# stardist/stardist

Measured on AMD Instinct MI355X. Metric: predict_instances() Mpix/s (2D) + Mvox/s (3D) end-to-end at 1/2/4/8 GPU, higher is better.
Workload: dtype f32

## Files before the change

include/stardist_hip.h:

```cpp
#ifndef STARDIST_HIP_H
#define STARDIST_HIP_H

#include <stdbool.h>
#include <stdint.h>

#ifdef __cplusplus
extern "C" {
#endif

const char* sd_last_error(void);
int sd_version(void);
int sd_device_count(void);
int sd_release_workspace(void);
int sd_set_option(const char* name, int value);
int sd_get_option(const char* name);

int sd_nms2d_host(const float* dist, const float* points, int n_polys, int n_rays,
                  int use_kdtree, int use_bbox, int verbose, float threshold,
                  uint8_t* keep, int64_t* stats);
int sd_nms2d_device(const float* d_dist, const float* d_points, int n_polys, int n_rays,
                    int use_kdtree, int use_bbox, int verbose, float threshold,
                    uint8_t* d_keep, int64_t* stats, void* stream);

int sd_nms2d_build_device(const float* d_dist, const float* d_points, int n_polys, int n_rays, int32_t* d_vx, int32_t* d_vy,
                          int32_t* d_bbox, float* d_radius, float* d_area, int32_t* d_gstats, void* stream);

int sd_nms2d_old_host(const int32_t* polys, int n_polys, int n_rays, const int32_t* mapping, int height, int width,
                      float threshold, int max_bbox_search, int grid_y, int grid_x, int verbose, uint8_t* keep);
int sd_nms2d_old_device(const int32_t* d_polys, int n_polys, int n_rays, const int32_t* d_mapping, int height, int width,
                        float threshold, int max_bbox_search, int grid_y, int grid_x, int verbose, uint8_t* d_keep, void* stream);

int sd_prepare_polys_device(const int32_t* d_x, const int32_t* d_y, int n_polys, int n_verts, void* d_out,
                            int64_t out_bytes, void* stream);

int sd_clip_pairs_device(const int32_t* d_xa, const int32_t* d_ya, const int32_t* d_xb,
                         const int32_t* d_yb, int n_pairs, int n_verts,
                         int64_t* d_out_twice_area, int32_t* d_out_flags, void* stream);

int sd_area_bounds_pairs_device(const int32_t* d_xa, const int32_t* d_ya, const int32_t* d_xb, const int32_t* d_yb, int n_pairs,
                                int n_verts, float* d_out_area, float* d_out_band, int32_t* d_out_info, void* stream);

int sd_poly_pass_device(const int32_t* d_x, const int32_t* d_y, int n_polys, int n_verts, void* d_props, void* d_prep, void* stream);

int sd_star_dist2d_host(const uint16_t* src, int H, int W, int n_rays, int grid_y, int grid_x,
                        float* dst);
int sd_star_dist2d_device(const uint16_t* d_src, int H, int W, int n_rays, int grid_y,
                          int grid_x, float* d_dst, void* stream);
int sd_star_dist3d_host(const uint16_t* src, int Z, int Y, int X, const float* dz,
                        const float* dy, const float* dx, int n_rays, int grid_z, int grid_y,
                        int grid_x, float* dst);
int sd_star_dist3d_device(const uint16_t* d_src, int Z, int Y, int X, const float* d_dz,
                          const float* d_dy, const float* d_dx, int n_rays, int grid_z,
                          int grid_y, int grid_x, float* d_dst, void* stream);

int sd_edt_prob_device(const int32_t* d_lbl, int Z, int Y, int X, double sz, double sy, double sx, int max_label,
                       float* d_prob, void* stream);

int sd_polygons_to_label_host(const float* coord, const int32_t* labels, int n_polys, int n_rays,
                              int H, int W, int32_t* result);
int sd_polygons_to_label_device(const float* d_coord, const int32_t* d_labels, int n_polys,
                                int n_rays, int H, int W, int32_t* d_result, void* stream);
int sd_polygons_to_label_window_device(const float* d_coord, const int32_t* d_labels, int n_polys, int n_rays, int HI, int WI,
                                       int y0, int x0, int H, int W, int32_t* d_result, void* stream);
// ... 182 lines not shown
```

stardist_amd/csrc/area_bounds.h:

```cpp
#pragma once
#include <hip/hip_runtime.h>

namespace sdarea {

enum { PP_PLAIN = 1, PP_POS = 2, PP_NEG = 4 };
struct PolyProps { float lmax, perim; int flags; int xmin, xmax, ymin, ymax; int pad; };

__device__ __forceinline__ float sgnf(float v) { return v > 0.f ? 1.f : (v < 0.f ? -1.f : 0.f); }
__device__ __forceinline__ float half_sum(float v) { for (int o = 16; o; o >>= 1) v += __shfl_xor(v, o); return v; }
__device__ __forceinline__ float half_max(float v) { for (int o = 16; o; o >>= 1) v = fmaxf(v, __shfl_xor(v, o)); return v; }
__device__ __forceinline__ int half_sum_i(int v) { for (int o = 16; o; o >>= 1) v += __shfl_xor(v, o); return v; }
__device__ __forceinline__ int half_min_i(int v) { for (int o = 16; o; o >>= 1) { const int t = __shfl_xor(v, o); v = t < v ? t : v; } return v; }
__device__ __forceinline__ int half_max_i(int v) { for (int o = 16; o; o >>= 1) { const int t = __shfl_xor(v, o); v = t > v ? t : v; } return v; }

constexpr float NEAR_W = 0.15f, STRIP_W = 0.45f;
constexpr int WINDOW = 2047;


struct Enclosure { float area, band; int crossings, near; bool usable; };

__device__ __forceinline__ Enclosure pair_enclosure(const int* __restrict__ px, const int* __restrict__ py, const int* __restrict__ qx,
                                                    const int* __restrict__ qy, int R, const PolyProps& pp, const PolyProps& pq, bool active,
                                                    float2* sq, int l, int half) {
  Enclosure E; E.area = 0.f; E.band = 0.f; E.crossings = 0; E.near = 0; E.usable = false;
  const int hb = half << 5;
  bool use = active && (pp.flags & PP_PLAIN) && (pq.flags & PP_PLAIN) && ((pp.flags & (PP_POS | PP_NEG)) == (pq.flags & (PP_POS | PP_NEG)));
  const int ox = use ? (int)(((long long)pp.xmin + pp.xmax) >> 1) : 0, oy = use ? (int)(((long long)pp.ymin + pp.ymax) >> 1) : 0;
  long long ext = 0;
  if (use) {
    const long long e0 = (long long)pp.xmax - ox, e1 = (long long)ox - pp.xmin, e2 = (long long)pp.ymax - oy, e3 = (long long)oy - pp.ymin;
    const long long e4 = (long long)pq.xmax - ox, e5 = (long long)ox - pq.xmin, e6 = (long long)pq.ymax - oy, e7 = (long long)oy - pq.ymin;
    ext = e0; ext = e1 > ext ? e1 : ext; ext = e2 > ext ? e2 : ext; ext = e3 > ext ? e3 : ext;
    ext = e4 > ext ? e4 : ext; ext = e5 > ext ? e5 : ext; ext = e6 > ext ? e6 : ext; ext = e7 > ext ? e7 : ext;
    if (ext > WINDOW / 2) use = false;
  }
  const bool lv = use && l < R;
  float ax = 0.f, ay = 0.f, cqx = 0.f, cqy = 0.f;
  if (lv) { ax = (float)(px[l] - ox); ay = (float)(py[l] - oy); cqx = (float)(qx[l] - ox); cqy = (float)(qy[l] - oy); }
  sq[l] = make_float2(cqx, cqy);
  const int ln = (l + 1 >= R) ? 0 : l + 1;
  const float bx = __shfl(ax, hb + ln), by = __shfl(ay, hb + ln);
  __builtin_amdgcn_wave_barrier();
  const float ex = bx - ax, ey = by - ay;
  const bool oke = lv && (ex != 0.f || ey != 0.f);
  const bool tie_e_pos = ey != 0.f ? ey < 0.f : ex > 0.f;
  const bool e_up = by > ay;
  const bool sPpos = (pp.flags & PP_POS) != 0, sQpos = (pq.flags & PP_POS) != 0;
  const float exlo = fminf(ax, bx) - 1.f, exhi = fmaxf(ax, bx) + 1.f, eylo = fminf(ay, by) - 1.f, eyhi = fmaxf(ay, by) + 1.f;
  float accP = 0.f, accQ = 0.f;
  int K = 0, T = 0, parA = 0, SQ = 0;
  bool nearP = false;
  float2 c = sq[0];
  float o_ec = ex * (c.y - ay) - ey * (c.x - ax);
  const int Rw = __any(use) ? R : 0;
  for (int k = 0; k < Rw; ++k) {
    const int kn = (k + 1 >= R) ? 0 : k + 1;
    const float2 d = sq[kn];
    const float fx = d.x - c.x, fy = d.y - c.y;
    const bool okf = use & ((fx != 0.f) | (fy != 0.f));
    const bool tie_f_pos = fy != 0.f ? fy > 0.f : fx < 0.f;
    const float o_ed = ex * (d.y - ay) - ey * (d.x - ax);
    const float o_fa = fx * (ay - c.y) - fy * (ax - c.x), o_fb = fx * (by - c.y) - fy * (bx - c.x);
    const bool pos_c = (o_ec > 0.f) | ((o_ec == 0.f) & tie_e_pos), pos_d = (o_ed > 0.f) | ((o_ed == 0.f) & tie_e_pos);
    const bool pos_a = (o_fa > 0.f) | ((o_fa == 0.f) & tie_f_pos), pos_b = (o_fb > 0.f) | ((o_fb == 0.f) & tie_f_pos);
    const float ccd = c.x * d.y - c.y * d.x;
    const bool both = oke & okf;
    const bool nearb = both & ((c.x <= exhi) | (d.x <= exhi)) & ((c.x >= exlo) | (d.x >= exlo)) & ((c.y <= eyhi) | (d.y <= eyhi)) & ((c.y >= eylo) | (d.y >= eylo));
    T += nearb ? 1 : 0;
    nearP |= nearb;
    {
      const unsigned long long nb64 = __ballot(nearb);
      SQ += ((unsigned int)(half ? (nb64 >> 32) : nb64) != 0u) ? 1 : 0;
    }
    if (both & (pos_c != pos_d) & (pos_a != pos_b)) {
      const float t = o_fa * __builtin_amdgcn_rcpf(o_fa - o_fb), u = o_ec * __builtin_amdgcn_rcpf(o_ec - o_ed);
      const float wt = 1.f - t, wu = 1.f - u;
      accP += (pos_b == sQpos) ? wt : -wt;
      accQ += ccd * ((pos_d == sPpos) ? wu : -wu);
      ++K;
    }
    parA ^= (okf & ((c.y < ay) != (d.y < ay)) & (pos_a == (fy > 0.f))) ? 1 : 0;
    const bool hitC = oke & use & ((ay <= c.y) != (by <= c.y)) & (pos_c == e_up);
    const unsigned long long hb64 = __ballot(hitC);
    const unsigned int hm = (unsigned int)(half ? (hb64 >> 32) : hb64);
    if ((__popc(hm) & 1) && l == 0) accQ += ccd;
    c = d; o_ec = o_ed;
  }
  const float cab = ax * by - ay * bx;
  const float contrib = lv ? cab * ((float)parA + accP) + accQ : 0.f;
  const float tot = half_sum(contrib);
  const int Kt = half_sum_i(lv ? K : 0), Tt = half_sum_i(lv ? T : 0), SPt = half_sum_i((lv && nearP) ? 1 : 0);
  const int St = SPt > SQ ? SPt : SQ;
  E.area = 0.5f * fabsf(tot);
  E.crossings = Kt; E.near = Tt;
  E.band = (0.5f * (float)Kt + fmaxf(NEAR_W * (float)Tt, STRIP_W * (float)St)) * (pp.lmax + pq.lmax) + 0.75f + 2e-6f * (float)ext * (pp.perim + pq.perim);
  if (use) {
    long long M = 0;
    const long long a0 = pp.xmin < 0 ? -(long long)pp.xmin : pp.xmin, a1 = pp.xmax < 0 ? -(long long)pp.xmax : pp.xmax;
    const long long a2 = pp.ymin < 0 ? -(long long)pp.ymin : pp.ymin, a3 = pp.ymax < 0 ? -(long long)pp.ymax : pp.ymax;
    const long long b0 = pq.xmin < 0 ? -(long long)pq.xmin : pq.xmin, b1 = pq.xmax < 0 ? -(long long)pq.xmax : pq.xmax;
    const long long b2 = pq.ymin < 0 ? -(long long)pq.ymin : pq.ymin, b3 = pq.ymax < 0 ? -(long long)pq.ymax : pq.ymax;
    M = (a0 > a1 ? a0 : a1); M = b0 > M ? b0 : M; M = b1 > M ? b1 : M;
    long long My = (a2 > a3 ? a2 : a3); My = b2 > My ? b2 : My; My = b3 > My ? b3 : My;
    const double bound = (double)(M + My + 2) * ((double)pp.perim + (double)pq.perim + 3.0 * Kt + 4.0);
    if (!(bound < 16777216.0)) use = false;
  }
  E.usable = use;
  return E;
}

__device__ __forceinline__ int decide(const Enclosure& E, float area_i, float area_j, float thr) {
  if (!E.usable) return 0;
  const double amin = fmin((double)area_i + 1.e-10, (double)area_j + 1.e-10);
  if (!(amin > 0.25)) return 0;
  const double lo = ((double)E.area - (double)E.band) / amin, hi = ((double)E.area + (double)E.band) / amin;
  const double m = 4e-6 * fabs((double)thr) + 1e-6;
  if (lo > (double)thr + m) return 2;
  if (hi < (double)thr - m) return 1;
  return 0;
}

}
```

stardist_amd/csrc/area_bounds.hip:

```cpp
#include "common.h"
#include "area_bounds.h"
#include "poly_pass.h"
#include "../../include/stardist_hip.h"

namespace {
__global__ void __launch_bounds__(256) k_area_probe(const int* __restrict__ xa, const int* __restrict__ ya, const int* __restrict__ xb,
                                                    const int* __restrict__ yb, int n, int R, const sdarea::PolyProps* __restrict__ pa,
                                                    const sdarea::PolyProps* __restrict__ pb, float* __restrict__ out_area, float* __restrict__ out_band,
                                                    int* __restrict__ out_info) {
  __shared__ float2 sq[4][2][32];
  const int lane = threadIdx.x & 63, half = lane >> 5, l = lane & 31, wv = threadIdx.x >> 6;
  const long long nw = (long long)gridDim.x * 4;
  for (long long base = 2ll * ((long long)blockIdx.x * 4 + wv); base < n; base += 2ll * nw) {
    const long long t = base + half;
    const bool active = t < n;
    const long long tt = active ? t : 0;
    const sdarea::Enclosure E = sdarea::pair_enclosure(xa + tt * R, ya + tt * R, xb + tt * R, yb + tt * R, R, pa[tt], pb[tt], active, sq[wv][half], l, half);
    if (active && l == 0) { out_area[t] = E.area; out_band[t] = E.band; out_info[t] = (E.usable ? 1 : 0) | ((E.crossings & 0x3FF) << 8) | ((E.near & 0x7FF) << 18); }
    __builtin_amdgcn_wave_barrier();
  }
}
}

extern "C" int sd_area_bounds_pairs_device(const int32_t* d_xa, const int32_t* d_ya, const int32_t* d_xb, const int32_t* d_yb, int n_pairs, int n_verts,
                                           float* d_out_area, float* d_out_band, int32_t* d_out_info, void* stream) {
  hipStream_t s = (hipStream_t)stream;
  if (n_pairs <= 0) return 0;
  const int R = n_verts;
  if (R < 3 || R > 32) { sd::set_error("sd_area_bounds_pairs: n_verts=%d unsupported (3..32)", R); return -1; }
  sd::Arena& A = sd::arena();
  if (A.begin(s)) return -1;
  sdarea::PolyProps* pa = (sdarea::PolyProps*)A.take((size_t)n_pairs * sizeof(sdarea::PolyProps));
  sdarea::PolyProps* pb = (sdarea::PolyProps*)A.take((size_t)n_pairs * sizeof(sdarea::PolyProps));
  if (!pa || !pb) return -1;
  if (sdpass::launch_poly_pass(d_xa, d_ya, n_pairs, R, pa, nullptr, s) || sdpass::launch_poly_pass(d_xb, d_yb, n_pairs, R, pb, nullptr, s)) {
    sd::set_error("sd_area_bounds_pairs: launch failed");
    return -1;
  }
  const int blocks = sd::div_up(n_pairs, 8) < 2048 ? sd::div_up(n_pairs, 8) : 2048;
  hipLaunchKernelGGL(k_area_probe, dim3(blocks), dim3(256), 0, s, d_xa, d_ya, d_xb, d_yb, n_pairs, R, pa, pb, d_out_area, d_out_band, d_out_info);
  SD_LAUNCH_CHECK();
  SD_CHECK(hipStreamSynchronize(s));
  return 0;
}

extern "C" int sd_poly_pass_device(const int32_t* d_x, const int32_t* d_y, int n_polys, int n_verts, void* d_props, void* d_prep, void* stream) {
  hipStream_t s = (hipStream_t)stream;
  if (n_polys <= 0 || (!d_props && !d_prep)) return 0;
  const int R = n_verts;
  if (R < (d_props ? 3 : 1) || R > 32) { sd::set_error("sd_poly_pass: n_verts=%d unsupported (%d..32)", R, d_props ? 3 : 1); return -1; }
  if (sdpass::launch_poly_pass(d_x, d_y, n_polys, R, (sdarea::PolyProps*)d_props, d_prep, s)) { sd::set_error("sd_poly_pass: launch failed"); return -1; }
  SD_CHECK(hipStreamSynchronize(s));
  return 0;
}
```

stardist_amd/csrc/common.h:

```cpp
#pragma once
#include <hip/hip_runtime.h>
#include <stdint.h>
#include <stdio.h>
#include <string.h>

namespace sd {

char* err_buf();
void set_error(const char* fmt, ...);

#define SD_CHECK(expr)                                                                   \
  do {                                                                                   \
    hipError_t _e = (expr);                                                              \
    if (_e != hipSuccess) {                                                              \
      sd::set_error("%s:%d: %s -> %s", __FILE__, __LINE__, #expr, hipGetErrorString(_e)); \
      return -1;                                                                         \
    }                                                                                    \
  } while (0)

#define SD_LAUNCH_CHECK() SD_CHECK(hipGetLastError())

class Arena {
 public:
  int begin(hipStream_t stream);
  void* take(size_t bytes);
  template <typename T> T* take_n(size_t n) { return (T*)take((n ? n : 1) * sizeof(T)); }
  void release();
  size_t capacity() const;
 private:
  enum { kMaxChunks = 64 };
  void* base_[kMaxChunks] = {};
  size_t cap_[kMaxChunks] = {};
  int n_ = 0, cur_ = 0;
  size_t off_ = 0;
};
Arena& arena();

hipStream_t side_stream();

static inline int div_up(long long a, long long b) { return (int)((a + b - 1) / b); }

enum Option { OPT_NMS3D_VOLUME_BOUNDS, OPT_NMS3D_CONE_MAP, OPT_NMS3D_REFINE_MESH, OPT_PROBE_TIER, OPT_PROBE_NO_GENERAL, OPT_TRACE, OPT_NMS3D_TAIL_BATCH, OPT_NMS3D_SPLIT_EXACT, OPT_CONV_F16_WGS, OPT_NMS2D_PAIR_LANES, OPT_NMS2D_AREA_BOUNDS, OPT_NMS2D_DEFER_UNDECIDED, OPT_NMS2D_STRICT, OPT_NMS2D_NBR_SINGLE, OPT_NMS3D_NBR_SINGLE, OPT_NMS2D_DEFER_MAX, OPT_NMS3D_BOUNDS_REUSE, OPT_NMS3D_DEFER_EXACT, OPT_NMS3D_BOUNDS_LEAN, OPT_COUNT };
int option(Option o);

#ifdef SD_DEBUG_SWITCHES
int tuning_env(const char* name, int dflt);
#else
static inline int tuning_env(const char*, int dflt) { return dflt; }
#endif

}
```

stardist_amd/csrc/lib.hip:

```cpp
#include "common.h"
#include "../../include/stardist_hip.h"
#include <stdarg.h>
#include <stdlib.h>
#include <mutex>

namespace sd {

static thread_local char g_err[1024] = "";
char* err_buf() { return g_err; }
void set_error(const char* fmt, ...) {
  va_list ap;
  va_start(ap, fmt);
  vsnprintf(g_err, sizeof(g_err), fmt, ap);
  va_end(ap);
}

static int g_opt[OPT_COUNT] = {1, 1, 2, 1, 0, 0, 1, 3, 2, 64, 1, 2, 0, 1, 1, 16384, 1, 3, 1};
static const char* const g_opt_name[OPT_COUNT] = {"nms3d_volume_bounds", "nms3d_cone_map", "nms3d_refine_mesh", "probe_tier", "probe_no_general", "trace", "nms3d_tail_batch", "nms3d_split_exact", "conv_f16_workgroups_per_cu", "nms2d_pair_lanes", "nms2d_area_bounds", "nms2d_defer_undecided", "nms2d_strict", "nms2d_neighbours_single_pass", "nms3d_neighbours_single_pass", "nms2d_defer_max", "nms3d_bounds_reuse", "nms3d_defer_exact", "nms3d_bounds_lean"};
int option(Option o) { return g_opt[o]; }
#ifdef SD_DEBUG_SWITCHES
int tuning_env(const char* name, int dflt) { const char* e = getenv(name); return e ? atoi(e) : dflt; }
#endif

enum { kMaxDevices = 64 };
static Arena g_arena[kMaxDevices];
Arena& arena() {
  int d = 0;
  if (hipGetDevice(&d) != hipSuccess || d < 0 || d >= kMaxDevices) d = 0;
  return g_arena[d];
}

hipStream_t side_stream() {
  static std::mutex mu;
  static hipStream_t st[kMaxDevices] = {};
  int d = 0;
  if (hipGetDevice(&d) != hipSuccess || d < 0 || d >= kMaxDevices) { set_error("side_stream: no current device"); return nullptr; }
  std::lock_guard<std::mutex> lock(mu);
  if (!st[d] && hipStreamCreateWithFlags(&st[d], hipStreamNonBlocking) != hipSuccess) { st[d] = nullptr; set_error("side_stream: cannot create a stream"); }
  return st[d];
}

size_t Arena::capacity() const { size_t t = 0; for (int i = 0; i < n_; ++i) t += cap_[i]; return t; }
int Arena::begin(hipStream_t stream) {
  if (n_ > 1) {
    size_t total = capacity();
    SD_CHECK(hipStreamSynchronize(stream));
    for (int i = 0; i < n_; ++i) { (void)hipFree(base_[i]); base_[i] = nullptr; cap_[i] = 0; }
    n_ = 0;
    size_t want = total + (total >> 3);
    SD_CHECK(hipMalloc(&base_[0], want));
    cap_[0] = want; n_ = 1;
  }
  cur_ = 0; off_ = 0;
  return 0;
}
void* Arena::take(size_t bytes) {
  for (;;) {
    if (cur_ < n_) {
      size_t a = (off_ + 255) & ~size_t(255);
      if (a + bytes <= cap_[cur_]) { off_ = a + bytes; return (char*)base_[cur_] + a; }
      ++cur_; off_ = 0;
      continue;
// ... 38 lines not shown
```

stardist_amd/csrc/nms2d.hip:

```cpp
#include <type_traits>

#include "common.h"
#include "clip_sweep.h"
#include "clip_beam.h"
#include "area_bounds.h"
#include "poly_pass.h"
#include "nms_rounds.h"
#include "../../include/stardist_hip.h"
#include <hipcub/hipcub.hpp>
#include <math.h>
#include <stdlib.h>
#include <vector>

namespace {

using sdclip::i64;

__device__ __forceinline__ float wave_min(float v) { for (int o = 32; o; o >>= 1) v = fminf(v, __shfl_xor(v, o)); return v; }
__device__ __forceinline__ float wave_max(float v) { for (int o = 32; o; o >>= 1) v = fmaxf(v, __shfl_xor(v, o)); return v; }
__device__ __forceinline__ i64 wave_sum(i64 v) { for (int o = 32; o; o >>= 1) v += __shfl_xor(v, o); return v; }

__global__ void __launch_bounds__(256) k_build(const float* __restrict__ dist, const float* __restrict__ pts,
                                               const float2* __restrict__ sincos, int N, int R,
                                               int* __restrict__ vx, int* __restrict__ vy, int4* __restrict__ bbox,
// ... 375 lines not shown
      continue;
    }
    if ((st & ~sdclip::ST_FAIL) || bm.n_joins > 0 || bm.sum_abs_terms >= (1ll << 24)) {
      const unsigned int k = atomicAdd(q.exactCount, 1u);
      if (k < q.cap) q.exact[k] = p;
      continue;
    }
    const float area_inter = 0.5f * (float)twice;
    const float overlap = (float)((double)area_inter / fmin((double)area[ij.x] + 1.e-10, (double)area[ij.y] + 1.e-10));
    if (overlap > thr) { if (supp) supp[p] = 1; else state[ij.y] = ST_SUPPRESSED; }
  }
}
template <int MAXV, int K, int MAXIL, int MAXREC, int S, bool REL16 = false>
size_t beam_lds_bytes() {
  typedef typename std::conditional<REL16, sdclip::LdsStorage16<S>, sdclip::LdsStorage<S>>::type Storage;
  return (size_t)sdclip::Beam<MAXV, K, MAXIL, MAXREC, Storage>::lds_bytes() + 64;
}

__global__ void __launch_bounds__(256) k_pairs_decide(const int2* __restrict__ pairs, const unsigned long long* __restrict__ nPtr,
                                                      const unsigned int* __restrict__ firstPtr, const int* __restrict__ vx, const int* __restrict__ vy, int R,
                                                      const sdarea::PolyProps* __restrict__ props, const float* __restrict__ area, float thr,
                                                      unsigned char* __restrict__ state, unsigned char* __restrict__ supp,
                                                      unsigned char* __restrict__ decided, unsigned int* __restrict__ nDecided) {
  __shared__ float2 sq[4][2][32];
  const int lane = threadIdx.x & 63, half = lane >> 5, l = lane & 31, wv = threadIdx.x >> 6;
  const unsigned long long n = *nPtr, first = firstPtr ? (unsigned long long)*firstPtr : 0ull;
  const unsigned long long nw = (unsigned long long)gridDim.x * 4;
  unsigned int mine = 0;
  for (unsigned long long base = first + 2ull * ((unsigned long long)blockIdx.x * 4 + wv); base < n; base += 2ull * nw) {
    const unsigned long long t = base + half;
    const bool active = t < n;
    const int2 ij = active ? pairs[t] : make_int2(0, 0);
    const sdarea::PolyProps pp = props[ij.x], pq = props[ij.y];
    const sdarea::Enclosure E = sdarea::pair_enclosure(vx + (size_t)ij.x * R, vy + (size_t)ij.x * R, vx + (size_t)ij.y * R, vy + (size_t)ij.y * R, R, pp, pq,
                                                       active, sq[wv][half], l, half);
    if (active && l == 0) {
      const int dec = sdarea::decide(E, area[ij.x], area[ij.y], thr);
      decided[t] = (unsigned char)dec;
      if (dec == 2) { if (supp) supp[t] = 1; else state[ij.y] = ST_SUPPRESSED; }
      if (dec) ++mine;
    }
    __builtin_amdgcn_wave_barrier();
  }
  mine += __shfl_xor(mine, 32);
  if (lane == 0 && mine) atomicAdd(nDecided, mine);
}

__global__ void __launch_bounds__(256) k_tail_emit(const int* __restrict__ U, int nU, const unsigned char* __restrict__ state,
                                                   const i64* __restrict__ nbrStart, const int* __restrict__ nbrLow, const int* __restrict__ nbr, NmsFlags f,
                                                   const float* __restrict__ pts, const int4* __restrict__ bbox,
                                                   const float* __restrict__ radius, const float* __restrict__ area,
                                                   int2* __restrict__ pairs, unsigned long long* pairCount, unsigned long long pairCap,
                                                   unsigned int* __restrict__ segStart, int* __restrict__ segCnt) {
  const int wave = threadIdx.x >> 6, lane = threadIdx.x & 63;
  for (int w = blockIdx.x * (blockDim.x >> 6) + wave; w < nU; w += gridDim.x * (blockDim.x >> 6)) {
    const int j = U[w];
    int cnt = 0;
    unsigned long long base = 0;
// ... 470 lines not shown
  const int* nbr = L.nbr;
  int* waitOn = L.waitOn;
  const i64 totalNbr = 2 * L.total;

  SD_CHECK(hipStreamWaitEvent(s, evProps, 0));
  if (stats) { SD_CHECK(hipEventRecord(ev1, s)); SD_CHECK(hipEventSynchronize(ev1)); float ms = 0; SD_CHECK(hipEventElapsedTime(&ms, ev0, ev1)); ns_pre = ms * 1e6; }

  const unsigned long long pairCap = (unsigned long long)(totalNbr / 2 + 64);
  int* U1 = A.take_n<int>(N);
  int* K = A.take_n<int>(N);
  int2* pairs = A.take_n<int2>(pairCap);
  const unsigned int qCap = (unsigned int)(pairCap < (1ull << 30) ? pairCap : (1ull << 30));
  unsigned int* spillPairs = A.take_n<unsigned int>(qCap);
  unsigned int* exactPairs = A.take_n<unsigned int>(qCap);
  int* Sl = A.take_n<int>(N);
  Counters* d_cnt = (Counters*)A.take(sizeof(Counters));
  static const bool pairSort = sd::tuning_env("SD_NMS_PAIR_SORT", 1) != 0;
  unsigned int* pairOrder = pairSort && R <= 32 ? A.take_n<unsigned int>(qCap) : nullptr;
  unsigned int* bucketHist = A.take_n<unsigned int>(2 * PAIR_BUCKETS);
  unsigned long long* nOrdered = A.take_n<unsigned long long>(1);
  if (!U0 || !U1 || !K || !pairs || !spillPairs || !exactPairs || !Sl || !d_cnt || !bucketHist || !nOrdered || (pairSort && R <= 32 && !pairOrder)) return -1;
  unsigned char* decided = (areaBounds && pairOrder) ? A.take_n<unsigned char>(pairCap) : nullptr;
  if (areaBounds && pairOrder && !decided) return -1;
  i64 totalDecided = 0, totalSkipped = 0;
  int nU = N, rounds = 0;
  i64 totalPairs = 0, totalExact = 0, totalSpill = 0;
  int* Ucur = U0; int* Unext = U1;
  Counters h;
  hipEvent_t ev2 = nullptr, ev3 = nullptr;
  if (stats) { SD_CHECK(hipEventCreate(&ev2)); SD_CHECK(hipEventCreate(&ev3)); }
  EvGuard evguard2{ev2, ev3};
  static const int tailDiv = sd::tuning_env("SD_NMS_TAIL_DIV", 6);
  static const int tailMax = sd::tuning_env("SD_NMS_TAIL_MAX", 65536);
  const int tailT = tailDiv > 0 ? ((N / tailDiv) < tailMax ? (N / tailDiv) : tailMax) : -1;
  unsigned char* supp = nullptr; unsigned int* segStart = nullptr; int* segCnt = nullptr;
  static const bool deferEnv = sd::tuning_env("SD_NMS_DEFER", 1) != 0;
  const bool deferOn = tailT >= 0 && deferEnv;
  Deferred dfr{nullptr, nullptr, nullptr, nullptr, nullptr, qCap};
  unsigned int* firstNew = A.take_n<unsigned int>(1);
  dfr.pend = pend0; dfr.head = head0; dfr.count = dcount0;
  if (!firstNew) return -1;
  if (deferOn) {
    dfr.pairs = A.take_n<int2>(qCap);
    dfr.next = A.take_n<int>(qCap);
    if (!dfr.pairs || !dfr.next) return -1;
  }
// ... 5 lines not shown
  const unsigned int deferMax = (unsigned int)(sd::option(sd::OPT_NMS2D_DEFER_MAX) > 0 ? sd::option(sd::OPT_NMS2D_DEFER_MAX) : 0);
  unsigned char* defKind = nullptr; unsigned int* nJoinDef = nullptr;
  if (deferFrom > 0) {
    defKind = A.take_n<unsigned char>(qCap); nJoinDef = A.take_n<unsigned int>(1);
    if (!defKind || !nJoinDef) return -1;
    SD_CHECK(hipMemsetAsync(defKind, 0, qCap, s));
  }
  i64 totalUndecDeferred = 0;
  i64 nUndecDeferredUpper = 0;
  auto run_pairs = [&](unsigned char* suppOut) -> int {
    const unsigned int* first = suppOut ? firstNew : nullptr;
    if (stats) SD_CHECK(hipEventRecord(ev0, s));
    PairQueues q1{spillPairs, &d_cnt->nSpill, exactPairs, &d_cnt->nExact, qCap};
    PairQueues q2{exactPairs, &d_cnt->nExact, exactPairs, &d_cnt->nExact, qCap};
    int rc;
    if (R <= 32) {
      if (pairOrder) {
        static const int keyMode = sd::tuning_env("SD_NMS_PAIR_KEY", 2);
        static const int modes[6][3] = {{1, 32, 32}, {1, 64, 16}, {1, 64, 64}, {16, 16, 16}, {16, 32, 8}, {4, 32, 32}};
        const int* md = modes[keyMode >= 0 && keyMode < 6 ? keyMode : 2];
        const PairKey key{(const char*)prep, prepStride, 1.f / (4.f * (max_dist + 1.f)), md[0], md[1], md[2]};
        SD_CHECK(hipMemsetAsync(bucketHist, 0, PAIR_BUCKETS * sizeof(unsigned int), s));
        if (decided)
          hipLaunchKernelGGL(k_pairs_decide, dim3(256 * 8), dim3(256), 0, s, pairs, &d_cnt->nPairs, first, vx, vy, R, props, area, threshold, state, suppOut,
                             decided, &d_cnt->nDecided);
        if (!suppOut && deferFrom > 0 && rounds >= deferFrom)
          hipLaunchKernelGGL(k_defer_undecided, dim3(256), dim3(256), 0, s, pairs, &d_cnt->nPairs, &d_cnt->nDecided, deferMax, decided, state, dfr, defKind, &d_cnt->nErr);
        const unsigned int* bfirst = (suppOut && deferFrom > 0) ? nullptr : first;
        SD_CHECK(hipStreamWaitEvent(s, evPrep, 0));
        const unsigned char* liveState = suppOut ? nullptr : state;
        hipLaunchKernelGGL(k_pair_bucket_count, dim3(512), dim3(256), 0, s, pairs, &d_cnt->nPairs, bfirst, d_points, key, bucketHist, decided, liveState,
                           &d_cnt->nSkipped);
        hipLaunchKernelGGL(k_pair_bucket_scan, dim3(1), dim3(1024), 0, s, bucketHist, bucketHist + PAIR_BUCKETS, nOrdered);
        hipLaunchKernelGGL(k_pair_bucket_scatter, dim3(512), dim3(256), 0, s, pairs, &d_cnt->nPairs, bfirst, d_points, key, bucketHist + PAIR_BUCKETS,
                           pairOrder, qCap, decided, liveState);
        SD_LAUNCH_CHECK();
        rc = BeamPath<32, 64>::tier1(pairs, pairOrder, nOrdered, (const unsigned int*)nullptr, prep, area, threshold, state, suppOut, q1, s);
      } else {
        SD_CHECK(hipStreamWaitEvent(s, evPrep, 0));
        rc = BeamPath<32, 64>::tier1(pairs, (const unsigned int*)nullptr, &d_cnt->nPairs, first, prep, area, threshold, state, suppOut, q1, s);
      }
      if (stats) SD_CHECK(hipEventRecord(ev1, s));
      if (!rc) rc = BeamPath<32, 64>::tier2(pairs, spillPairs, &d_cnt->nSpill, (const unsigned int*)nullptr, prep, area, threshold, state, suppOut, q2, s);
    } else {
      SD_CHECK(hipStreamWaitEvent(s, evPrep, 0));
      if (R <= 64) rc = BeamPath<64, 64>::tier2(pairs, (const unsigned int*)nullptr, &d_cnt->nPairs, first, prep, area, threshold, state, suppOut, q2, s);
      else if (R <= 128) rc = BeamPath<128, 32>::tier2(pairs, (const unsigned int*)nullptr, &d_cnt->nPairs, first, prep, area, threshold, state, suppOut, q2, s);
// ... 323 lines not shown
```

stardist_amd/lib/_native.py:

```python
import ctypes
import os

import numpy as np

_HERE = os.path.dirname(os.path.abspath(__file__))
LIB_PATH = os.path.join(_HERE, "..", "csrc", "libstardist_hip.so")

_lib = None
last_stats = {}

_c_f32p = ctypes.POINTER(ctypes.c_float)
_c_i32p = ctypes.POINTER(ctypes.c_int32)
_c_i64p = ctypes.POINTER(ctypes.c_int64)
_c_u8p = ctypes.POINTER(ctypes.c_uint8)
_c_u16p = ctypes.POINTER(ctypes.c_uint16)
_vp = ctypes.c_void_p
_i = ctypes.c_int
_f = ctypes.c_float

SIGNATURES = {
    "sd_last_error": (ctypes.c_char_p, []),
    "sd_version": (_i, []),
    "sd_device_count": (_i, []),
    "sd_release_workspace": (_i, []),
    "sd_set_option": (_i, [ctypes.c_char_p, _i]),
    "sd_get_option": (_i, [ctypes.c_char_p]),
    "sd_nms2d_host": (_i, [_vp, _vp, _i, _i, _i, _i, _i, _f, _vp, _vp]),
    "sd_nms2d_device": (_i, [_vp, _vp, _i, _i, _i, _i, _i, _f, _vp, _vp, _vp]),
    "sd_nms2d_build_device": (_i, [_vp, _vp, _i, _i, _vp, _vp, _vp, _vp, _vp, _vp, _vp]),
    "sd_nms2d_old_host": (_i, [_vp, _i, _i, _vp, _i, _i, _f, _i, _i, _i, _i, _vp]),
    "sd_nms2d_old_device": (_i, [_vp, _i, _i, _vp, _i, _i, _f, _i, _i, _i, _i, _vp, _vp]),
    "sd_clip_pairs_device": (_i, [_vp, _vp, _vp, _vp, _i, _i, _vp, _vp, _vp]),
    "sd_area_bounds_pairs_device": (_i, [_vp, _vp, _vp, _vp, _i, _i, _vp, _vp, _vp, _vp]),
    "sd_prepare_polys_device": (_i, [_vp, _vp, _i, _i, _vp, ctypes.c_int64, _vp]),
    "sd_poly_pass_device": (_i, [_vp, _vp, _i, _i, _vp, _vp, _vp]),
    "sd_star_dist2d_host": (_i, [_vp, _i, _i, _i, _i, _i, _vp]),
    "sd_star_dist2d_device": (_i, [_vp, _i, _i, _i, _i, _i, _vp, _vp]),
    "sd_star_dist3d_host": (_i, [_vp, _i, _i, _i, _vp, _vp, _vp, _i, _i, _i, _i, _vp]),
    "sd_star_dist3d_device": (_i, [_vp, _i, _i, _i, _vp, _vp, _vp, _i, _i, _i, _i, _vp, _vp]),
    "sd_edt_prob_device": (_i, [_vp, _i, _i, _i, ctypes.c_double, ctypes.c_double, ctypes.c_double, _i, _vp, _vp]),
    "sd_dist_to_coord_device": (_i, [_vp, _vp, _vp, ctypes.c_longlong, _i, ctypes.c_double, ctypes.c_double, _vp, _vp]),
    "sd_polygons_to_label_host": (_i, [_vp, _vp, _i, _i, _i, _i, _vp]),
    "sd_polygons_to_label_device": (_i, [_vp, _vp, _i, _i, _i, _i, _vp, _vp]),
    "sd_polygons_to_label_window_device": (_i, [_vp, _vp, _i, _i, _i, _i, _i, _i, _i, _i, _vp, _vp]),
    "sd_polyhedron_to_label_window_device": (_i, [_vp, _vp, _vp, _vp, _i, _i, _i, _vp] + [_i] * 13 + [_vp, _vp]),
    "_LIB_non_maximum_suppression_sparse": (None, [_vp, _vp, _vp, _i, _i, _i, _vp, _vp, _f, _i, _i, _i, _vp]),
    "sd_nms3d_device": (_i, [_vp, _vp, _vp, _i, _i, _i, _vp, _vp, _f, _i, _i, _i, _vp, _vp, _vp]),
    "sd_hiv_pairs_device": (_i, [_vp, _vp, _i, _i, _i, _vp, _vp, _vp, _i, _vp, _vp, _vp]),
    "_LIB_polyhedron_to_label": (None, [_vp, _vp, _vp, _vp, _i, _i, _i, _vp, _i, _i, _i, _i, _i, _i, _i, _vp]),
    "sd_polyhedron_to_label_device": (_i, [_vp, _vp, _vp, _vp, _i, _i, _i, _vp, _i, _i, _i, _i, _i, _i, _i, _vp, _vp]),
    "sd_select_candidates_device": (_i, [_vp, _vp, _i, _vp, _vp, _i, _f, _i, _vp, _vp, _vp, _vp, _vp]),
    "sd_survivor_positions_device": (_i, [_vp, ctypes.c_longlong, _vp, _vp, _vp]),
    "sd_survivors2d_device": (_i, [_vp, _i, _vp, _vp, _vp, _i, _vp, _vp, _vp, _vp, _vp, _vp, _vp]),
    "sd_sorted_rows_device": (_i, [_vp, _vp, _i, _i, _vp, _vp, _vp, _vp, _vp, _vp, _vp]),
    "sd_sort_scores_desc_device": (_i, [_vp, _i, _vp, _vp, _vp]),
    "sd_bias_act_device": (_i, [_vp, _vp, ctypes.c_longlong, _i, ctypes.c_longlong, _i, _vp]),
# ... 138 lines not shown
```

Before: 322.0.

## Restructure pair enclosure inner loop with precomputed edge records and lane masks

```diff
diff --git a/include/stardist_hip.h b/include/stardist_hip.h
--- a/include/stardist_hip.h
+++ b/include/stardist_hip.h
@@ -39,6 +39,7 @@
 
 int sd_area_bounds_pairs_device(const int32_t* d_xa, const int32_t* d_ya, const int32_t* d_xb, const int32_t* d_yb, int n_pairs,
                                 int n_verts, float* d_out_area, float* d_out_band, int32_t* d_out_info, void* stream);
+int sd_area_bounds_pairs_grid(void);
 
 int sd_poly_pass_device(const int32_t* d_x, const int32_t* d_y, int n_polys, int n_verts, void* d_props, void* d_prep, void* stream);
 
diff --git a/stardist_amd/csrc/area_bounds.h b/stardist_amd/csrc/area_bounds.h
--- a/stardist_amd/csrc/area_bounds.h
+++ b/stardist_amd/csrc/area_bounds.h
@@ -19,90 +19,140 @@
 
 struct Enclosure { float area, band; int crossings, near; bool usable; };
 
-__device__ __forceinline__ Enclosure pair_enclosure(const int* __restrict__ px, const int* __restrict__ py, const int* __restrict__ qx,
-                                                    const int* __restrict__ qy, int R, const PolyProps& pp, const PolyProps& pq, bool active,
-                                                    float2* sq, int l, int half) {
+struct PairOperands { int word, px, py, qx, qy; };
+__device__ __forceinline__ PairOperands load_operands(const int* __restrict__ px, const int* __restrict__ py, const int* __restrict__ qx,
+                                                      const int* __restrict__ qy, const PolyProps* __restrict__ pp, const PolyProps* __restrict__ pq,
+                                                      bool live, int l) {
+  static_assert(sizeof(PolyProps) == 32, "eight words per record");
+  PairOperands o;
+  o.word = 0;
+  if (l < 16) o.word = (l < 8 ? (const int*)pp : (const int*)pq)[l & 7];
+  o.px = o.py = o.qx = o.qy = 0;
+  if (live) { o.px = px[l]; o.py = py[l]; o.qx = qx[l]; o.qy = qy[l]; }
+  return o;
+}
+__device__ __forceinline__ PolyProps props_from_lanes(int word, int first) {
+  PolyProps p;
+  p.lmax = __int_as_float(__shfl(word, first)); p.perim = __int_as_float(__shfl(word, first + 1)); p.flags = __shfl(word, first + 2);
+  p.xmin = __shfl(word, first + 3); p.xmax = __shfl(word, first + 4); p.ymin = __shfl(word, first + 5); p.ymax = __shfl(word, first + 6);
+  p.pad = 0;
+  return p;
+}
+
+typedef unsigned long long lanemask;
+__device__ __forceinline__ lanemask lanes_where(bool p) { return __builtin_amdgcn_ballot_w64(p); }
+__device__ __forceinline__ bool my_lane(lanemask m) { return __builtin_amdgcn_inverse_ballot_w64(m); }
+__device__ __forceinline__ unsigned int lower(lanemask m) { return (unsigned int)m; }
+__device__ __forceinline__ unsigned int upper(lanemask m) { return (unsigned int)(m >> 32); }
+__device__ __forceinline__ float cross_plus(float a, float b, float c, float d, float h) { return __fmaf_rn(a, b, __fmaf_rn(-c, d, h)); }
+__device__ __forceinline__ int half_or_i(int v) { for (int o = 16; o; o >>= 1) v |= __shfl_xor(v, o); return v; }
+
+enum { REC_ROWS = 3, REC_FLOAT4 = REC_ROWS * 32 };
+
+__device__ __forceinline__ Enclosure pair_enclosure(const PairOperands& o, int R, bool active, float4* rec, int l, int half) {
+  const int hb = half << 5;
   Enclosure E; E.area = 0.f; E.band = 0.f; E.crossings = 0; E.near = 0; E.usable = false;
-  const int hb = half << 5;
-  bool use = active && (pp.flags & PP_PLAIN) && (pq.flags & PP_PLAIN) && ((pp.flags & (PP_POS | PP_NEG)) == (pq.flags & (PP_POS | PP_NEG)));
-  const int ox = use ? (int)(((long long)pp.xmin + pp.xmax) >> 1) : 0, oy = use ? (int)(((long long)pp.ymin + pp.ymax) >> 1) : 0;
+  const PolyProps pp0 = props_from_lanes(o.word, hb), pq0 = props_from_lanes(o.word, hb + 8);
+  bool use = active && (pp0.flags & PP_PLAIN) && (pq0.flags & PP_PLAIN) && ((pp0.flags & (PP_POS | PP_NEG)) == (pq0.flags & (PP_POS | PP_NEG)));
+  const int ox = use ? (int)(((long long)pp0.xmin + pp0.xmax) >> 1) : 0, oy = use ? (int)(((long long)pp0.ymin + pp0.ymax) >> 1) : 0;
   long long ext = 0;
   if (use) {
-    const long long e0 = (long long)pp.xmax - ox, e1 = (long long)ox - pp.xmin, e2 = (long long)pp.ymax - oy, e3 = (long long)oy - pp.ymin;
-    const long long e4 = (long long)pq.xmax - ox, e5 = (long long)ox - pq.xmin, e6 = (long long)pq.ymax - oy, e7 = (long long)oy - pq.ymin;
+    const long long e0 = (long long)pp0.xmax - ox, e1 = (long long)ox - pp0.xmin, e2 = (long long)pp0.ymax - oy, e3 = (long long)oy - pp0.ymin;
+    const long long e4 = (long long)pq0.xmax - ox, e5 = (long long)ox - pq0.xmin, e6 = (long long)pq0.ymax - oy, e7 = (long long)oy - pq0.ymin;
     ext = e0; ext = e1 > ext ? e1 : ext; ext = e2 > ext ? e2 : ext; ext = e3 > ext ? e3 : ext;
     ext = e4 > ext ? e4 : ext; ext = e5 > ext ? e5 : ext; ext = e6 > ext ? e6 : ext; ext = e7 > ext ? e7 : ext;
     if (ext > WINDOW / 2) use = false;
   }
+  const float extf = (float)ext;
+  const bool sPpos = (pp0.flags & PP_POS) != 0, sQpos = (pq0.flags & PP_POS) != 0;
   const bool lv = use && l < R;
   float ax = 0.f, ay = 0.f, cqx = 0.f, cqy = 0.f;
-  if (lv) { ax = (float)(px[l] - ox); ay = (float)(py[l] - oy); cqx = (float)(qx[l] - ox); cqy = (float)(qy[l] - oy); }
-  sq[l] = make_float2(cqx, cqy);
+  if (lv) { ax = (float)(o.px - ox); ay = (float)(o.py - oy); cqx = (float)(o.qx - ox); cqy = (float)(o.qy - oy); }
   const int ln = (l + 1 >= R) ? 0 : l + 1;
-  const float bx = __shfl(ax, hb + ln), by = __shfl(ay, hb + ln);
+  const float bxs = __shfl(ax, hb + ln), bys = __shfl(ay, hb + ln);
+  const float bx = lv ? bxs : ax, by = lv ? bys : ay;
+  const float INF = __builtin_huge_valf();
+  {
+    const float dqx = __shfl(cqx, hb + ln), dqy = __shfl(cqy, hb + ln);
+    const float fx = dqx - cqx, fy = dqy - cqy;
+    const bool okf = use & ((fx != 0.f) | (fy != 0.f));
+    const bool tie_f_pos = fy != 0.f ? fy > 0.f : fx < 0.f;
+    rec[l] = make_float4(cqx, cqy, dqx, dqy);
+    rec[32 + l] = make_float4(fx, fy, cqx * dqy - cqy * dqx, tie_f_pos ? 0.5f : -0.5f);
+    rec[64 + l] = okf ? make_float4(fminf(cqx, dqx), fmaxf(cqx, dqx), fminf(cqy, dqy), fmaxf(cqy, dqy)) : make_float4(INF, -INF, INF, -INF);
+  }
   __builtin_amdgcn_wave_barrier();
   const float ex = bx - ax, ey = by - ay;
   const bool oke = lv && (ex != 0.f || ey != 0.f);
-  const bool tie_e_pos = ey != 0.f ? ey < 0.f : ex > 0.f;
-  const bool e_up = by > ay;
-  const bool sPpos = (pp.flags & PP_POS) != 0, sQpos = (pq.flags & PP_POS) != 0;
-  const float exlo = fminf(ax, bx) - 1.f, exhi = fmaxf(ax, bx) + 1.f, eylo = fminf(ay, by) - 1.f, eyhi = fmaxf(ay, by) + 1.f;
+  const float h_e = (ey != 0.f ? ey < 0.f : ex > 0.f) ? 0.5f : -0.5f;
+  const lanemask m_e_up = lanes_where(by > ay), m_sP = lanes_where(sPpos), m_sQ = lanes_where(sQpos);
+  const float exlo = oke ? fminf(ax, bx) - 1.f : INF, exhi = oke ? fmaxf(ax, bx) + 1.f : -INF;
+  const float eylo = oke ? fminf(ay, by) - 1.f : INF, eyhi = oke ? fmaxf(ay, by) + 1.f : -INF;
+  const float cab = ax * by - ay * bx;
   float accP = 0.f, accQ = 0.f;
-  int K = 0, T = 0, parA = 0, SQ = 0;
-  bool nearP = false;
-  float2 c = sq[0];
-  float o_ec = ex * (c.y - ay) - ey * (c.x - ax);
+  int K = 0;
+  unsigned int nearbits = 0;
+  lanemask m_parA = 0;
+  float4 q0 = rec[0], q1 = rec[32], q2 = rec[64];
+  float dcx = q0.x - ax, dcy = q0.y - ay;
+  float o_ec = cross_plus(ex, dcy, ey, dcx, h_e);
+  lanemask m_pos_c = lanes_where(o_ec > 0.f), m_c_lt_a = lanes_where(q0.y < ay), m_c_lt_b = lanes_where(q0.y < by);
   const int Rw = __any(use) ? R : 0;
-  for (int k = 0; k < Rw; ++k) {
+  auto edge = [&](int k, const float4& q0, const float4& q1, const float4& q2, float4& n0, float4& n1, float4& n2) {
     const int kn = (k + 1 >= R) ? 0 : k + 1;
-    const float2 d = sq[kn];
-    const float fx = d.x - c.x, fy = d.y - c.y;
-    const bool okf = use & ((fx != 0.f) | (fy != 0.f));
-    const bool tie_f_pos = fy != 0.f ? fy > 0.f : fx < 0.f;
-    const float o_ed = ex * (d.y - ay) - ey * (d.x - ax);
-    const float o_fa = fx * (ay - c.y) - fy * (ax - c.x), o_fb = fx * (by - c.y) - fy * (bx - c.x);
-    const bool pos_c = (o_ec > 0.f) | ((o_ec == 0.f) & tie_e_pos), pos_d = (o_ed > 0.f) | ((o_ed == 0.f) & tie_e_pos);
-    const bool pos_a = (o_fa > 0.f) | ((o_fa == 0.f) & tie_f_pos), pos_b = (o_fb > 0.f) | ((o_fb == 0.f) & tie_f_pos);
-    const float ccd = c.x * d.y - c.y * d.x;
-    const bool both = oke & okf;
-    const bool nearb = both & ((c.x <= exhi) | (d.x <= exhi)) & ((c.x >= exlo) | (d.x >= exlo)) & ((c.y <= eyhi) | (d.y <= eyhi)) & ((c.y >= eylo) | (d.y >= eylo));
-    T += nearb ? 1 : 0;
-    nearP |= nearb;
-    {
-      const unsigned long long nb64 = __ballot(nearb);
-      SQ += ((unsigned int)(half ? (nb64 >> 32) : nb64) != 0u) ? 1 : 0;
-    }
-    if (both & (pos_c != pos_d) & (pos_a != pos_b)) {
-      const float t = o_fa * __builtin_amdgcn_rcpf(o_fa - o_fb), u = o_ec * __builtin_amdgcn_rcpf(o_ec - o_ed);
+    n0 = rec[kn]; n1 = rec[32 + kn]; n2 = rec[64 + kn];
+    const float fx = q1.x, fy = q1.y, ccd = q1.z, h_f = q1.w;
+    const float ddx = q0.z - ax, ddy = q0.w - ay;
+    const float o_ed = cross_plus(ex, ddy, ey, ddx, h_e);
+    const float o_fa = cross_plus(fy, dcx, fx, dcy, h_f);
+    const float o_fb = o_fa + __fmaf_rn(fx, ey, -(fy * ex));
+    const lanemask m_pos_d = lanes_where(o_ed > 0.f), m_pos_a = lanes_where(o_fa > 0.f), m_pos_b = lanes_where(o_fb > 0.f);
+    const bool nearb = (q2.x <= exhi) & (q2.y >= exlo) & (q2.z <= eyhi) & (q2.w >= eylo);
+    nearbits |= nearb ? 1u << k : 0u;
+    if (my_lane((m_pos_c ^ m_pos_d) & (m_pos_a ^ m_pos_b))) {
+      const float r_f = o_fa - h_f, r_c = o_ec - h_e;
+      const float t = r_f * __builtin_amdgcn_rcpf(o_fa - o_fb), u = r_c * __builtin_amdgcn_rcpf(o_ec - o_ed);
       const float wt = 1.f - t, wu = 1.f - u;
-      accP += (pos_b == sQpos) ? wt : -wt;
-      accQ += ccd * ((pos_d == sPpos) ? wu : -wu);
+      accP += my_lane(~(m_pos_b ^ m_sQ)) ? wt : -wt;
+      accQ += ccd * (my_lane(~(m_pos_d ^ m_sP)) ? wu : -wu);
       ++K;
     }
-    parA ^= (okf & ((c.y < ay) != (d.y < ay)) & (pos_a == (fy > 0.f))) ? 1 : 0;
-    const bool hitC = oke & use & ((ay <= c.y) != (by <= c.y)) & (pos_c == e_up);
-    const unsigned long long hb64 = __ballot(hitC);
-    const unsigned int hm = (unsigned int)(half ? (hb64 >> 32) : hb64);
-    if ((__popc(hm) & 1) && l == 0) accQ += ccd;
-    c = d; o_ec = o_ed;
+    const lanemask m_d_lt_a = lanes_where(q0.w < ay), m_d_lt_b = lanes_where(q0.w < by);
+    m_parA ^= (m_c_lt_a ^ m_d_lt_a) & ~(m_pos_a ^ lanes_where(fy > 0.f));
+    const lanemask m_hit = (m_c_lt_a ^ m_c_lt_b) & ~(m_pos_c ^ m_e_up);
+    const lanemask m_odd = (lanemask)(__popc(lower(m_hit)) & 1) | ((lanemask)(__popc(upper(m_hit)) & 1) << 32);
+    if (my_lane(m_odd)) accQ += ccd;
+    dcx = ddx; dcy = ddy; o_ec = o_ed; m_pos_c = m_pos_d; m_c_lt_a = m_d_lt_a; m_c_lt_b = m_d_lt_b;
+  };
+  float4 p0, p1, p2;
+  int k = 0;
+  for (; k + 1 < Rw; k += 2) {
+    edge(k, q0, q1, q2, p0, p1, p2);
+    edge(k + 1, p0, p1, p2, q0, q1, q2);
   }
-  const float cab = ax * by - ay * bx;
-  const float contrib = lv ? cab * ((float)parA + accP) + accQ : 0.f;
+  if (k < Rw) edge(k, q0, q1, q2, p0, p1, p2);
+  const float contrib = lv ? cab * ((my_lane(m_parA) ? 1.f : 0.f) + accP) + accQ : 0.f;
   const float tot = half_sum(contrib);
-  const int Kt = half_sum_i(lv ? K : 0), Tt = half_sum_i(lv ? T : 0), SPt = half_sum_i((lv && nearP) ? 1 : 0);
-  const int St = SPt > SQ ? SPt : SQ;
-  E.area = 0.5f * fabsf(tot);
-  E.crossings = Kt; E.near = Tt;
-  E.band = (0.5f * (float)Kt + fmaxf(NEAR_W * (float)Tt, STRIP_W * (float)St)) * (pp.lmax + pq.lmax) + 0.75f + 2e-6f * (float)ext * (pp.perim + pq.perim);
-  if (use) {
-    long long M = 0;
+  const PolyProps pp = props_from_lanes(o.word, hb), pq = props_from_lanes(o.word, hb + 8);
+  const float lsum = pp.lmax + pq.lmax, fterm = 2e-6f * extf * (pp.perim + pq.perim);
+  const double psum = (double)pp.perim + (double)pq.perim;
+  long long MM = 0;
+  {
     const long long a0 = pp.xmin < 0 ? -(long long)pp.xmin : pp.xmin, a1 = pp.xmax < 0 ? -(long long)pp.xmax : pp.xmax;
     const long long a2 = pp.ymin < 0 ? -(long long)pp.ymin : pp.ymin, a3 = pp.ymax < 0 ? -(long long)pp.ymax : pp.ymax;
     const long long b0 = pq.xmin < 0 ? -(long long)pq.xmin : pq.xmin, b1 = pq.xmax < 0 ? -(long long)pq.xmax : pq.xmax;
     const long long b2 = pq.ymin < 0 ? -(long long)pq.ymin : pq.ymin, b3 = pq.ymax < 0 ? -(long long)pq.ymax : pq.ymax;
-    M = (a0 > a1 ? a0 : a1); M = b0 > M ? b0 : M; M = b1 > M ? b1 : M;
+    long long M = (a0 > a1 ? a0 : a1); M = b0 > M ? b0 : M; M = b1 > M ? b1 : M;
     long long My = (a2 > a3 ? a2 : a3); My = b2 > My ? b2 : My; My = b3 > My ? b3 : My;
-    const double bound = (double)(M + My + 2) * ((double)pp.perim + (double)pq.perim + 3.0 * Kt + 4.0);
+    MM = M + My + 2;
+  }
+  const int Kt = half_sum_i(K), Tt = half_sum_i(__popc(nearbits)), SPt = half_sum_i(nearbits != 0u ? 1 : 0), SQ = __popc((unsigned int)half_or_i((int)nearbits));
+  const int St = SPt > SQ ? SPt : SQ;
+  E.area = 0.5f * fabsf(tot);
+  E.crossings = Kt; E.near = Tt;
+  E.band = (0.5f * (float)Kt + fmaxf(NEAR_W * (float)Tt, STRIP_W * (float)St)) * lsum + 0.75f + fterm;
+  if (use) {
+    const double bound = (double)MM * (psum + 3.0 * Kt + 4.0);
     if (!(bound < 16777216.0)) use = false;
   }
   E.usable = use;
diff --git a/stardist_amd/csrc/area_bounds.hip b/stardist_amd/csrc/area_bounds.hip
--- a/stardist_amd/csrc/area_bounds.hip
+++ b/stardist_amd/csrc/area_bounds.hip
@@ -8,18 +8,28 @@
                                                     const int* __restrict__ yb, int n, int R, const sdarea::PolyProps* __restrict__ pa,
                                                     const sdarea::PolyProps* __restrict__ pb, float* __restrict__ out_area, float* __restrict__ out_band,
                                                     int* __restrict__ out_info) {
-  __shared__ float2 sq[4][2][32];
+  __shared__ float4 rec[4][2][sdarea::REC_FLOAT4];
   const int lane = threadIdx.x & 63, half = lane >> 5, l = lane & 31, wv = threadIdx.x >> 6;
-  const long long nw = (long long)gridDim.x * 4;
-  for (long long base = 2ll * ((long long)blockIdx.x * 4 + wv); base < n; base += 2ll * nw) {
+  const long long step = 2ll * gridDim.x * 4;
+  for (long long base = 2ll * ((long long)blockIdx.x * 4 + wv); base < n; base += step) {
     const long long t = base + half;
     const bool active = t < n;
     const long long tt = active ? t : 0;
-    const sdarea::Enclosure E = sdarea::pair_enclosure(xa + tt * R, ya + tt * R, xb + tt * R, yb + tt * R, R, pa[tt], pb[tt], active, sq[wv][half], l, half);
+    const sdarea::PairOperands o = sdarea::load_operands(xa + tt * R, ya + tt * R, xb + tt * R, yb + tt * R, pa + tt, pb + tt, active && l < R, l);
+    const sdarea::Enclosure E = sdarea::pair_enclosure(o, R, active, rec[wv][half], l, half);
     if (active && l == 0) { out_area[t] = E.area; out_band[t] = E.band; out_info[t] = (E.usable ? 1 : 0) | ((E.crossings & 0x3FF) << 8) | ((E.near & 0x7FF) << 18); }
     __builtin_amdgcn_wave_barrier();
   }
 }
+int probe_grid() {
+  static int cache[sd::kMaxDevices] = {};
+  return sd::resident_grid((const void*)k_area_probe, 256, cache);
+}
+}
+
+extern "C" int sd_area_bounds_pairs_grid(void) {
+  const int g = probe_grid();
+  return g > 0 ? g : -1;
 }
 
 extern "C" int sd_area_bounds_pairs_device(const int32_t* d_xa, const int32_t* d_ya, const int32_t* d_xb, const int32_t* d_yb, int n_pairs, int n_verts,
@@ -28,6 +38,8 @@
   if (n_pairs <= 0) return 0;
   const int R = n_verts;
   if (R < 3 || R > 32) { sd::set_error("sd_area_bounds_pairs: n_verts=%d unsupported (3..32)", R); return -1; }
+  const int grid = probe_grid();
+  if (grid <= 0) return -1;
   sd::Arena& A = sd::arena();
   if (A.begin(s)) return -1;
   sdarea::PolyProps* pa = (sdarea::PolyProps*)A.take((size_t)n_pairs * sizeof(sdarea::PolyProps));
@@ -37,7 +49,7 @@
     sd::set_error("sd_area_bounds_pairs: launch failed");
     return -1;
   }
-  const int blocks = sd::div_up(n_pairs, 8) < 2048 ? sd::div_up(n_pairs, 8) : 2048;
+  const int blocks = sd::div_up(n_pairs, 8) < grid ? sd::div_up(n_pairs, 8) : grid;
   hipLaunchKernelGGL(k_area_probe, dim3(blocks), dim3(256), 0, s, d_xa, d_ya, d_xb, d_yb, n_pairs, R, pa, pb, d_out_area, d_out_band, d_out_info);
   SD_LAUNCH_CHECK();
   SD_CHECK(hipStreamSynchronize(s));
diff --git a/stardist_amd/csrc/common.h b/stardist_amd/csrc/common.h
--- a/stardist_amd/csrc/common.h
+++ b/stardist_amd/csrc/common.h
@@ -38,6 +38,9 @@
 
 hipStream_t side_stream();
 
+enum { kMaxDevices = 64 };
+int resident_grid(const void* kernel, int threads, int* cache);
+
 static inline int div_up(long long a, long long b) { return (int)((a + b - 1) / b); }
 
 enum Option { OPT_NMS3D_VOLUME_BOUNDS, OPT_NMS3D_CONE_MAP, OPT_NMS3D_REFINE_MESH, OPT_PROBE_TIER, OPT_PROBE_NO_GENERAL, OPT_TRACE, OPT_NMS3D_TAIL_BATCH, OPT_NMS3D_SPLIT_EXACT, OPT_CONV_F16_WGS, OPT_NMS2D_PAIR_LANES, OPT_NMS2D_AREA_BOUNDS, OPT_NMS2D_DEFER_UNDECIDED, OPT_NMS2D_STRICT, OPT_NMS2D_NBR_SINGLE, OPT_NMS3D_NBR_SINGLE, OPT_NMS2D_DEFER_MAX, OPT_NMS3D_BOUNDS_REUSE, OPT_NMS3D_DEFER_EXACT, OPT_NMS3D_BOUNDS_LEAN, OPT_COUNT };
diff --git a/stardist_amd/csrc/lib.hip b/stardist_amd/csrc/lib.hip
--- a/stardist_amd/csrc/lib.hip
+++ b/stardist_amd/csrc/lib.hip
@@ -22,7 +22,6 @@
 int tuning_env(const char* name, int dflt) { const char* e = getenv(name); return e ? atoi(e) : dflt; }
 #endif
 
-enum { kMaxDevices = 64 };
 static Arena g_arena[kMaxDevices];
 Arena& arena() {
   int d = 0;
@@ -38,6 +37,23 @@
   std::lock_guard<std::mutex> lock(mu);
   if (!st[d] && hipStreamCreateWithFlags(&st[d], hipStreamNonBlocking) != hipSuccess) { st[d] = nullptr; set_error("side_stream: cannot create a stream"); }
   return st[d];
+}
+
+int resident_grid(const void* kernel, int threads, int* cache) {
+  static std::mutex mu;
+  int d = 0;
+  if (hipGetDevice(&d) != hipSuccess || d < 0 || d >= kMaxDevices) { set_error("resident_grid: no current device"); return 0; }
+  std::lock_guard<std::mutex> lock(mu);
+  if (!cache[d]) {
+    int per_cu = 0, cus = 0;
+    if (hipOccupancyMaxActiveBlocksPerMultiprocessor(&per_cu, kernel, threads, 0) != hipSuccess ||
+        hipDeviceGetAttribute(&cus, hipDeviceAttributeMultiprocessorCount, d) != hipSuccess || per_cu <= 0 || cus <= 0) {
+      set_error("resident_grid: occupancy query failed");
+      return 0;
+    }
+    cache[d] = per_cu * cus;
+  }
+  return cache[d];
 }
 
 size_t Arena::capacity() const { size_t t = 0; for (int i = 0; i < n_; ++i) t += cap_[i]; return t; }
diff --git a/stardist_amd/csrc/nms2d.hip b/stardist_amd/csrc/nms2d.hip
--- a/stardist_amd/csrc/nms2d.hip
+++ b/stardist_amd/csrc/nms2d.hip
@@ -421,18 +421,18 @@
                                                       const sdarea::PolyProps* __restrict__ props, const float* __restrict__ area, float thr,
                                                       unsigned char* __restrict__ state, unsigned char* __restrict__ supp,
                                                       unsigned char* __restrict__ decided, unsigned int* __restrict__ nDecided) {
-  __shared__ float2 sq[4][2][32];
+  __shared__ float4 rec[4][2][sdarea::REC_FLOAT4];
   const int lane = threadIdx.x & 63, half = lane >> 5, l = lane & 31, wv = threadIdx.x >> 6;
   const unsigned long long n = *nPtr, first = firstPtr ? (unsigned long long)*firstPtr : 0ull;
-  const unsigned long long nw = (unsigned long long)gridDim.x * 4;
+  const unsigned long long step = 2ull * gridDim.x * 4;
   unsigned int mine = 0;
-  for (unsigned long long base = first + 2ull * ((unsigned long long)blockIdx.x * 4 + wv); base < n; base += 2ull * nw) {
+  for (unsigned long long base = first + 2ull * ((unsigned long long)blockIdx.x * 4 + wv); base < n; base += step) {
     const unsigned long long t = base + half;
     const bool active = t < n;
     const int2 ij = active ? pairs[t] : make_int2(0, 0);
-    const sdarea::PolyProps pp = props[ij.x], pq = props[ij.y];
-    const sdarea::Enclosure E = sdarea::pair_enclosure(vx + (size_t)ij.x * R, vy + (size_t)ij.x * R, vx + (size_t)ij.y * R, vy + (size_t)ij.y * R, R, pp, pq,
-                                                       active, sq[wv][half], l, half);
+    const sdarea::PairOperands o = sdarea::load_operands(vx + (size_t)ij.x * R, vy + (size_t)ij.x * R, vx + (size_t)ij.y * R, vy + (size_t)ij.y * R,
+                                                         props + ij.x, props + ij.y, active && l < R, l);
+    const sdarea::Enclosure E = sdarea::pair_enclosure(o, R, active, rec[wv][half], l, half);
     if (active && l == 0) {
       const int dec = sdarea::decide(E, area[ij.x], area[ij.y], thr);
       decided[t] = (unsigned char)dec;
@@ -949,6 +949,9 @@
   if (!U0 || !U1 || !K || !pairs || !spillPairs || !exactPairs || !Sl || !d_cnt || !bucketHist || !nOrdered || (pairSort && R <= 32 && !pairOrder)) return -1;
   unsigned char* decided = (areaBounds && pairOrder) ? A.take_n<unsigned char>(pairCap) : nullptr;
   if (areaBounds && pairOrder && !decided) return -1;
+  static int decideGridOf[sd::kMaxDevices] = {};
+  const int decideGrid = decided ? sd::resident_grid((const void*)k_pairs_decide, 256, decideGridOf) : 0;
+  if (decided && decideGrid <= 0) return -1;
   i64 totalDecided = 0, totalSkipped = 0;
   int nU = N, rounds = 0;
   i64 totalPairs = 0, totalExact = 0, totalSpill = 0;
@@ -1000,7 +1003,7 @@
         const PairKey key{(const char*)prep, prepStride, 1.f / (4.f * (max_dist + 1.f)), md[0], md[1], md[2]};
         SD_CHECK(hipMemsetAsync(bucketHist, 0, PAIR_BUCKETS * sizeof(unsigned int), s));
         if (decided)
-          hipLaunchKernelGGL(k_pairs_decide, dim3(256 * 8), dim3(256), 0, s, pairs, &d_cnt->nPairs, first, vx, vy, R, props, area, threshold, state, suppOut,
+          hipLaunchKernelGGL(k_pairs_decide, dim3(decideGrid), dim3(256), 0, s, pairs, &d_cnt->nPairs, first, vx, vy, R, props, area, threshold, state, suppOut,
                              decided, &d_cnt->nDecided);
         if (!suppOut && deferFrom > 0 && rounds >= deferFrom)
           hipLaunchKernelGGL(k_defer_undecided, dim3(256), dim3(256), 0, s, pairs, &d_cnt->nPairs, &d_cnt->nDecided, deferMax, decided, state, dfr, defKind, &d_cnt->nErr);
diff --git a/stardist_amd/lib/_native.py b/stardist_amd/lib/_native.py
--- a/stardist_amd/lib/_native.py
+++ b/stardist_amd/lib/_native.py
@@ -32,6 +32,7 @@
     "sd_nms2d_old_device": (_i, [_vp, _i, _i, _vp, _i, _i, _f, _i, _i, _i, _i, _vp, _vp]),
     "sd_clip_pairs_device": (_i, [_vp, _vp, _vp, _vp, _i, _i, _vp, _vp, _vp]),
     "sd_area_bounds_pairs_device": (_i, [_vp, _vp, _vp, _vp, _i, _i, _vp, _vp, _vp, _vp]),
+    "sd_area_bounds_pairs_grid": (_i, []),
     "sd_prepare_polys_device": (_i, [_vp, _vp, _i, _i, _vp, ctypes.c_int64, _vp]),
     "sd_poly_pass_device": (_i, [_vp, _vp, _i, _i, _vp, _vp, _vp]),
     "sd_star_dist2d_host": (_i, [_vp, _i, _i, _i, _i, _i, _vp]),
```

Measured after the change: 334.6, median of 6. 1.04x the previous value.
